# JianCao92/speaker-diarization

Measured on AMD Instinct MI355X. Metric: diarized audio throughput (CD gw/BIC + CL hi/BIC), higher is better.
Workload: dtype f64

## Files before the change

speaker-diarization_amd/csrc/spkd_cd.hpp:

```cpp
#pragma once
#include <type_traits>
#include "spkd_device.hpp"
#include "spkd_quad.hpp"
#include "spkd_stats.hpp"
#include "spkd_cluster.hpp"
#include "../../include/spkd.h"

namespace spkd {

constexpr double NEG_MAXINT_M1 = -9223372036854775808.0;

struct TurnDesc {
    int64_t begin;
    int64_t len;
    int64_t cand_off;
    int64_t cand_cap;
    int64_t ev_off;
    int64_t ev_cap;
    int64_t id;
};

struct BestD {
    double d;
    long long k;
// ... 269 lines not shown
                load_fv<G::BR>(xi + f * DA, a);
                load_fv<G::BC>(xj + f * DA, b);
                frame(a, b);
            }
        }
        pos = stop;
    }
#ifdef SPKD_PROFILE
    SW_TICK(0);
    if (tid == 0) for (int i = 0; i < 3; ++i) atomicAdd(&g_gw_prof[8 + i], sw_acc[i]);
    if (tid == 0) atomicAdd(&g_gw_prof[11], sw_reached);
#endif
}

struct SweepOut {
    long long pos;
    double next_i;
    long long built_k;
};

template <int NW>
__device__ __noinline__ SweepOut gw_sweep_coarse(const float* __restrict__ fr, double* __restrict__ cache,
                                                 double start, double istep, double built_i,
                                                 long long built_k, long long cap, long long sweep_pos,
                                                 long long c, int fresh, int* err) {
    using G = Gw<NW>;
    extern __shared__ double gw_lds[];
    double* ldsEnd = gw_lds;
    float* xs = (float*)(gw_lds + TREC);
    const int tid = threadIdx.x;
    const SweepLane SL = sweep_lane<NW>(tid);
    const SPKD_GLOBAL float* gfr = (const SPKD_GLOBAL float*)fr;
    SPKD_GLOBAL double* gcache = (SPKD_GLOBAL double*)cache;
    double acc[G::NACC];
    if (fresh) {
#pragma unroll
        for (int e = 0; e < G::NACC; ++e) acc[e] = 0.0;
    } else {
        sweep_gather_lds<NW>(ldsEnd, SL, acc);
    }
    __syncthreads();
    auto next_stop = [&]() -> long long {
        const long long b = built_k < cap ? (long long)(start + built_i) : c;
        return b < c ? b : c;
    };
    gw_sweep<NW>(gfr, xs, SL, tid, acc, sweep_pos, next_stop(), c, [&](long long pos) -> long long {
        if (pos < c) {
            sweep_dump_packed<NW>(gcache + built_k * REC, SL, acc);
            ++built_k;
            built_i += istep;
            return next_stop();
        }
        sweep_dump_lds<NW>(ldsEnd, SL, acc);
        return -1;
    }, err);
    SweepOut o;
    o.pos = c;
    o.next_i = built_i;
    o.built_k = built_k;
    return o;
}

template <int NW>
__device__ __noinline__ void gw_sweep_fine(const float* __restrict__ fr, double* __restrict__ cache,
                                           const double* __restrict__ base, long long base_pos,
                                           double start, double fine_i0, long long F,
                                           long long first_slot, int* err) {
    using G = Gw<NW>;
    extern __shared__ double gw_lds[];
    float* xs = (float*)(gw_lds + TREC);
    const int tid = threadIdx.x;
    const SweepLane SL = sweep_lane<NW>(tid);
    const SPKD_GLOBAL float* gfr = (const SPKD_GLOBAL float*)fr;
    SPKD_GLOBAL double* gcache = (SPKD_GLOBAL double*)cache;
    double acc[G::NACC];
#pragma unroll
    for (int e = 0; e < G::NACC; ++e) acc[e] = 0.0;
    if (base) sweep_gather_packed<NW>((const SPKD_GLOBAL double*)base, SL, acc);
    double fx = fine_i0;
    long long fk = 0;
    const long long last = (long long)(start + (fine_i0 + (double)(F - 1)));
    gw_sweep<NW>(gfr, xs, SL, tid, acc, base_pos, (long long)(start + fx), last, [&](long long) -> long long {
        sweep_dump_packed<NW>(gcache + (first_slot + fk) * REC, SL, acc);
        ++fk;
        fx += 1;
        return fk < F ? (long long)(start + fx) : -1;
    }, err);
}

template <int NW>
__device__ __noinline__ void gw_sweep_tail(const float* __restrict__ fr, long long from, long long to,
                                           double* __restrict__ out, int* err) {
    using G = Gw<NW>;
    extern __shared__ double gw_lds[];
    float* xs = (float*)(gw_lds + TREC);
    const int tid = threadIdx.x;
    const SweepLane SL = sweep_lane<NW>(tid);
    const SPKD_GLOBAL float* gfr = (const SPKD_GLOBAL float*)fr;
    SPKD_GLOBAL double* gout = (SPKD_GLOBAL double*)out;
    double acc[G::NACC];
#pragma unroll
    for (int e = 0; e < G::NACC; ++e) acc[e] = 0.0;
    gw_sweep<NW>(gfr, xs, SL, tid, acc, from, to, to, [&](long long) -> long long {
        sweep_dump_packed<NW>(gout, SL, acc);
        return -1;
    }, err);
}

__device__ __forceinline__ void single_split_matrix(int pass, const double* ldsEnd,
                                                    const double* __restrict__ rec_b,
                                                    double n1, double n2, double (&q)[DA]) {
    const double n = n1 + n2;
    double rc[DA];
    if (pass == PASS_POOLED) {
        single_rows_from_tri(ldsEnd, q);
        cov_rows(q, n);
        return;
    }
    single_rows_from_packed(rec_b, q);
    if (pass == PASS_LEFT) {
        cov_rows(q, n1);
        return;
    }
    single_rows_from_tri(ldsEnd, rc);
    if (pass == PASS_RIGHT) {
#pragma unroll
        for (int j = 0; j < DA; ++j) q[j] = rc[j] - q[j];
        cov_rows(q, n2);
    } else {
        const double al1 = (n1 / n) / (n1 - 1.0), al2 = (n2 / n) / (n2 - 1.0);
        const double be1 = al1 / n1, be2 = al2 / n2;
        const double s1i = q[D], s2i = rc[D] - q[D];
#pragma unroll
        for (int j = 0; j < D; ++j) {
            const double q1 = q[j], q2 = rc[j] - q[j];
            const double s1j = readlane_d(s1i, j), s2j = readlane_d(s2i, j);
            double v = fma(al2, q2, al1 * q1);
            v = fma(-(be1 * s1i), s1j, v);
            q[j] = fma(-(be2 * s2i), s2j, v);
        }
    }
}

__device__ __forceinline__ double quad_split_det(int pass, bool two, const double* ldsEnd,
                                                    const double* __restrict__ rec_b,
                                                    double ik, double start, long long a, long long c,
                                                    const QuadLane& L, int* err) {
    QuadRows q;
    double svb[QS];
    PASS_T0();
    int ta = L.t;
    asm volatile("" : "+v"(ta));
    {
        const int t12 = ta < QL ? ta : QL - 1;
        const double* rt[2];
        long long o1 = 512;
        asm volatile("" : "+v"(o1));
        rt[0] = rec_b + t12;
        rt[1] = rt[0] + o1;
#pragma unroll
        for (int s = 0; s < QS; ++s) {
#pragma unroll
            for (int j = 0; j < tri_cols(s); ++j) {
                const int e = pk_off(j) + QL * s - j;
                q.r[s][j] = rt[e / 512][e % 512];
            }
            const int c = QL * s + t12;
            svb[s] = rec_b[pk_off(c) + D - c];
        }
    }
    __builtin_amdgcn_sched_barrier(0);
    const long long b = pass == PASS_POOLED ? a : (long long)(start + ik);
    const double n1 = (double)(b - a), n2 = (double)(c - b);
    const double n = n1 + n2;
    double al, ga, k1a, k1c, k2a, k2c, w1, w2;
    {
        const bool glr = two && pass == PASS_GLR;
        double al1 = 0.0, al2 = 0.0, b1 = 0.0, b2 = 0.0;
        if (two) {
            al1 = (n1 / n) / (n1 - 1.0);
            al2 = (n2 / n) / (n2 - 1.0);
            b1 = al1 / n1;
            b2 = al2 / n2;
        }
        const double np = pass == PASS_RIGHT ? n2 : (pass == PASS_LEFT ? n1 : n);
        const double f = fast_recip(np - 1.0);
        const double sa = pass == PASS_RIGHT ? -1.0 : (pass == PASS_LEFT ? 1.0 : 0.0);
        const double sg = pass == PASS_LEFT ? 0.0 : 1.0;
        al = glr ? al1 - al2 : sa * f;
        ga = glr ? al2 : sg * f;
        k1a = glr ? 1.0 : sa;
        k1c = glr ? 0.0 : sg;
        w1 = glr ? -b1 : -(f * fast_recip(np));
        k2a = glr ? -1.0 : 0.0;
        k2c = glr ? 1.0 : 0.0;
        w2 = glr ? -b2 : 0.0;
    }
    __builtin_amdgcn_sched_barrier(0);
    PASS_LOADED();
    double v1[QS], v2[QS], c1[QS], c2[QS];
#pragma unroll
    for (int s = 0; s < QS; ++s) {
#pragma unroll
        for (int j = 0; j < tri_cols(s); ++j)
            q.r[s][j] = fma(ga, ldsEnd[(tri_off(s) + j) * 16 + ta], al * q.r[s][j]);
        const double sc = ldsEnd[(TREC_SUMS + s) * 16 + ta];
        v1[s] = fma(k1c, sc, k1a * svb[s]);
        v2[s] = fma(k2c, sc, k2a * svb[s]);
        c1[s] = w1 * v1[s];
        c2[s] = w2 * v2[s];
        __builtin_amdgcn_sched_barrier(0);
    }
    TriRank1<0>::run(q, c1, v1);
    if (two) TriRank1<0>::run(q, c2, v2);
    auto form_single = [&](int mi, double (&arr)[DA]) {
        const double* rm = (const double*)__shfl((unsigned long long)rec_b, 16 * mi);
        single_split_matrix(__shfl(pass, 16 * mi), ldsEnd, rm, __shfl(n1, 16 * mi), __shfl(n2, 16 * mi), arr);
    };
    const double det = tri_det(q, L.m, err, form_single);
    PASS_DONE();
    return det;
}


#ifdef SPKD_PROFILE
#define GW_TICK(i) do { const unsigned long long now_ = clock64(); prof_acc[i] += now_ - prof_t; prof_t = now_; } while (0)
#else
#define GW_TICK(i) ((void)0)
#endif

struct GwState {
    double start, end, ws, dws, cur_i, built_i, maxd, maxi, fine_i0;
    long long n_memo;
    long long n_written;
    long long C;
    long long built_k, sweep_pos;
    int fresh;
    long long best_k, F, base, count;
    long long seg_src, seg_dst;
    int nw, nd;
    int next_q;
    int fine;
    int go;
    int abort;
    int tail_in_lds;
};

template <int NW>
__global__ __launch_bounds__(Gw<NW>::TPB, NW == 8 ? 1 : 2) void k_gw(
        const float* __restrict__ frames, const TurnDesc* __restrict__ turns, spkd_cd_params P,
        double* __restrict__ cache_all, double* __restrict__ cand_all,
        int32_t* __restrict__ n_win, double* __restrict__ win_maxd, int32_t* __restrict__ win_det,
        double* __restrict__ det_start, double* __restrict__ det_maxi, double* __restrict__ det_d,
        double* __restrict__ final_start, double* __restrict__ seg_stats, spkd_cand_log* clog,
        long long log_cap, unsigned long long* log_count, int* err,
        double* pinv_ws) {
    extern __shared__ double gw_lds[];
    double* ldsEnd = gw_lds;
    constexpr int GW_WAVES = NW, GW_TPB = Gw<NW>::TPB;
    __shared__ BestD red[GW_WAVES];
    __shared__ double s_ldS;
    __shared__ double s_common[2];
    __shared__ GwState S;
    const int tid = threadIdx.x, lane = lane_id(), wave = tid >> 6;
    const QuadLane L = quad_lane();
    const TurnDesc T = turns[blockIdx.x];
    const int turn = (int)T.id;
    const long long n = T.len;
    const float* fr = frames + T.begin * D;
    double* cache = cache_all + T.cand_off * REC;
    const long long cap = T.cand_cap;
    double* c_i = cand_all + 4 * T.cand_off;
    double* c_left = c_i + cap;
    double* c_x = c_left + cap;
    double* c_w = c_x + cap;

#ifdef SPKD_PROFILE
    unsigned long long prof_acc[4] = {0ull, 0ull, 0ull, 0ull}, prof_t = clock64(), prof_scans = 0ull;
    unsigned long long prof_passes = 0ull, prof_items = 0ull;
#endif
    for (int e = tid; e < TREC; e += GW_TPB) ldsEnd[e] = 0.0;
    for (int e = tid; e < REC; e += GW_TPB) cache[e] = 0.0;

    const int kind = P.kind;
    const double winsize = P.winsize, winstep = P.winstep, rate = P.rate;
    const double minfeas = rate / 2;
    const double istep = rate / 10;
    const double fn = (double)n;
    const double pen_w = P.lambdac * 0.5 * PEN_UNIT;
    if (tid == 0) {
        S.start = 0.0;
        S.end = winsize * 2;
        S.ws = minfeas;
        S.dws = P.deltaws;
        S.cur_i = minfeas;
        S.built_i = minfeas;
        S.maxd = 0.0; S.maxi = 0.0; S.fine_i0 = 0.0;
        S.n_memo = 0; S.n_written = 0; S.C = 0;
        S.built_k = 0; S.sweep_pos = 0; S.fresh = 1;
        S.best_k = 0; S.F = 0; S.base = 0; S.count = 0;
        S.seg_src = -1; S.seg_dst = -1;
        S.nw = 0; S.nd = 0; S.fine = 0;
        S.go = (S.end <= fn) ? 1 : 0;
        S.abort = 0;
        S.tail_in_lds = 0;
    }
    __syncthreads();
    GW_TICK(0);

    while (S.go) {
        if (tid == 0) {
            if (!S.fine) {
                if (S.nw >= T.ev_cap) {
                    atomicOr(err, 4);
                    S.abort = 1;
                } else {
                    const double lim = S.end - S.start - minfeas;
                    double cur_i = S.cur_i;
                    long long C = S.C, n_written = S.n_written;
                    while (cur_i < lim) {
// ... 430 lines not shown
```

speaker-diarization_amd/csrc/spkd_cluster.hpp:

```cpp
#pragma once
#include "spkd_device.hpp"
#include "spkd_quad.hpp"
#include "spkd_tri.hpp"
#include "../../include/spkd.h"

namespace spkd {

constexpr double MAXINT_F = 9223372036854775808.0;
constexpr double PEN_UNIT = 39.0 + 0.5 * 39.0 * 40.0;
constexpr int AUX = 3 * DA;
constexpr int ERR_DEGENERATE_MERGE = 2;

__device__ __forceinline__ unsigned long long dkey(double v) {
    unsigned long long b = (unsigned long long)__double_as_longlong(v);
    return (b >> 63) ? ~b : (b | 0x8000000000000000ull);
}
__device__ __forceinline__ double dkey_inv(unsigned long long k) {
    unsigned long long b = (k >> 63) ? (k & 0x7fffffffffffffffull) : ~k;
    return __longlong_as_double((long long)b);
}
template <bool MAXOP>
__device__ __forceinline__ unsigned wave_red_u32(unsigned x) {
    auto op = [](unsigned a, unsigned b) { return MAXOP ? (a > b ? a : b) : (a < b ? a : b); };
    x = op(x, (unsigned)__builtin_amdgcn_update_dpp((int)x, (int)x, 0xB1, 0xf, 0xf, false));
    x = op(x, (unsigned)__builtin_amdgcn_update_dpp((int)x, (int)x, 0x4E, 0xf, 0xf, false));
    x = op(x, (unsigned)__builtin_amdgcn_update_dpp((int)x, (int)x, 0x141, 0xf, 0xf, false));
    x = op(x, (unsigned)__builtin_amdgcn_update_dpp((int)x, (int)x, 0x140, 0xf, 0xf, false));
    const unsigned a = (unsigned)__builtin_amdgcn_readlane((int)x, 0), b = (unsigned)__builtin_amdgcn_readlane((int)x, 16);
    const unsigned c = (unsigned)__builtin_amdgcn_readlane((int)x, 32), d = (unsigned)__builtin_amdgcn_readlane((int)x, 48);
    return op(op(a, b), op(c, d));
}
__device__ __forceinline__ int wave_scan_i32(int x) {
    x += __builtin_amdgcn_update_dpp(0, x, 0x111, 0xf, 0xf, false);
    x += __builtin_amdgcn_update_dpp(0, x, 0x112, 0xf, 0xf, false);
    x += __builtin_amdgcn_update_dpp(0, x, 0x114, 0xf, 0xf, false);
    x += __builtin_amdgcn_update_dpp(0, x, 0x118, 0xf, 0xf, false);
    x += __builtin_amdgcn_update_dpp(0, x, 0x142, 0xa, 0xf, false);
    x += __builtin_amdgcn_update_dpp(0, x, 0x143, 0xc, 0xf, false);
    return x;
}
template <bool MAXOP>
__device__ __forceinline__ unsigned long long wave_red_u64(unsigned long long k) {
    const unsigned hi = (unsigned)(k >> 32), lo = (unsigned)k;
    const unsigned h = wave_red_u32<MAXOP>(hi);
    const unsigned l = wave_red_u32<MAXOP>(hi == h ? lo : (MAXOP ? 0u : 0xffffffffu));
    return ((unsigned long long)h << 32) | l;
}
__device__ __forceinline__ void wave_argmin_key(unsigned long long key, unsigned idx,
                                                unsigned long long& okey, unsigned& oidx) {
    okey = wave_red_u64<false>(key);
    oidx = wave_red_u32<false>(key == okey ? idx : 0xffffffffu);
}

__device__ __forceinline__ bool stat_valid(double d) {
    return d == d && fabs(d) < __builtin_huge_val();
}

__device__ __forceinline__ double kl2_combine(double s1, double p1, double m1,
                                              double s2, double p2, double m2);
__device__ __forceinline__ double kl2_from_aux(const double* __restrict__ a1,
                                               const double* __restrict__ a2) {
    int i = lane_id();
    i = i >= D ? D - 1 : i;
    return kl2_combine(a1[i], a1[DA + i], a1[2 * DA + i], a2[i], a2[DA + i], a2[2 * DA + i]);
}
__device__ __forceinline__ double kl2_from_aux_serial(const double* a1, const double* a2) {
    double t1 = 0.0, t2 = 0.0;
    for (int i = 0; i < D; ++i) {
        const float dm = (float)a1[2 * DA + i] - (float)a2[2 * DA + i];
        const double delta = (double)dm;
        t1 += (a1[i] - a2[i]) * (a2[DA + i] - a1[DA + i]);
        t2 += ((a1[DA + i] + a2[DA + i]) * delta) * delta;
    }
    return 0.5 * t1 + 0.5 * t2;
}

__device__ __forceinline__ void kl2_lane_terms(double (&a)[DA], double mean_i,
                                               double& ds, double& dp, double& mu, double* pinv_ws) {
    double out[2];
    spd_diag_terms_fn(a, out, pinv_ws);
    ds = out[0];
    dp = out[1];
    mu = (double)(float)mean_i;
}

__device__ __forceinline__ double kl2_combine(double s1, double p1, double m1,
                                              double s2, double p2, double m2) {
    const float dm = (float)m1 - (float)m2;
    const double delta = (double)dm;
    const double t1 = wave_sum39((s1 - s2) * (p2 - p1));
    const double t2 = wave_sum39(((p1 + p2) * delta) * delta);
    return 0.5 * t1 + 0.5 * t2;
}

constexpr int PT_WAVES = 4;

__device__ __forceinline__ void quadrec_from_packed(const double* __restrict__ g, double* __restrict__ o, int tid) {
    for (int e = tid; e < QREC; e += 256) {
        const int t = e & 15, sj = e >> 4;
        const int s = sj / DA, j = sj - s * DA;
        double v = 0.0;
        if (t < QL) {
            const int i = QL * s + t;
            const int r = i < j ? i : j, cc = i < j ? j : i;
            v = g[pk(r, cc)];
        } else if (e == QREC_COUNT_AT) {
            v = g[REC - 1];
        }
        o[e] = v;
    }
}

__global__ __launch_bounds__(256) void k_to_quadrec(const double* __restrict__ packed, int64_t n_rec,
                                                    double* __restrict__ qr) {
    const int64_t c = blockIdx.x;
    if (c >= n_rec) return;
    quadrec_from_packed(packed + c * REC, qr + c * QREC, threadIdx.x);
}

__device__ __forceinline__ void single_rows_from_packed(const double* __restrict__ rec, double (&q)[DA]) {
    int i = lane_id();
    i = i >= D ? D - 1 : i;
#pragma unroll
    for (int j = 0; j < D; ++j) q[j] = rec[j <= i ? pk_low(i, j) : pk_low(j, i)];
    q[D] = rec[pk_low(D, i)];
}

__device__ __forceinline__ void single_rows_from_qr(const double* __restrict__ qr, double (&q)[DA]) {
    int i = lane_id();
    i = i >= D ? D - 1 : i;
    const int base = (i / QL) * DA * 16 + (i % QL);
#pragma unroll
    for (int j = 0; j < DA; ++j) q[j] = qr[base + j * 16];
}

__device__ __forceinline__ void kl2_aux_from_qr(const double* qr, double* aux_out, double* pinv_ws) {
    double a[DA];
    single_rows_from_qr(qr, a);
    const double n = qr_count(qr);
    const double mean_i = a[D] / n;
    cov_rows(a, n);
    double ds, dp, mu;
    kl2_lane_terms(a, mean_i, ds, dp, mu, pinv_ws);
    const int lane = lane_id();
    if (lane < D) {
        aux_out[lane] = ds;
        aux_out[DA + lane] = dp;
        aux_out[2 * DA + lane] = mu;
    }
}

__device__ __forceinline__ void single_pair_matrix(int kind, const double* __restrict__ qrA,
                                                   const double* __restrict__ qrC, bool self,
                                                   double (&q)[DA]) {
    const double nA = qr_count(qrA);
    single_rows_from_qr(qrA, q);
    if (self) { cov_rows(q, nA); return; }
    const double nC = qr_count(qrC), n = nA + nC;
    double q2[DA];
    single_rows_from_qr(qrC, q2);
    if (kind == SPKD_BIC) {
#pragma unroll
        for (int j = 0; j < DA; ++j) q[j] += q2[j];
        cov_rows(q, n);
    } else {
        const double al1 = (nA / n) / (nA - 1.0), al2 = (nC / n) / (nC - 1.0);
        const double be1 = al1 / nA, be2 = al2 / nC;
        const double s1i = q[D], s2i = q2[D];
#pragma unroll
        for (int j = 0; j < D; ++j) {
            const double s1j = readlane_d(s1i, j), s2j = readlane_d(s2i, j);
            double v = fma(al2, q2[j], al1 * q[j]);
            v = fma(-(be1 * s1i), s1j, v);
            q[j] = fma(-(be2 * s2i), s2j, v);
        }
    }
}

#ifdef SPKD_PROFILE
__device__ unsigned long long g_pass_prof[4];
#define PASS_T0() const unsigned long long pass_t0_ = clock64()
#define PASS_LOADED() asm volatile("s_waitcnt vmcnt(0)" ::: "memory"); const unsigned long long pass_t1_ = clock64()
#define PASS_DONE() do { if (lane_id() == 0 && ((pass_t0_ >> 4) & 63) == 0) { const unsigned long long pass_t2_ = clock64();  \
        atomicAdd(&g_pass_prof[0], pass_t1_ - pass_t0_); atomicAdd(&g_pass_prof[1], pass_t2_ - pass_t0_); \
        atomicAdd(&g_pass_prof[2], 1ull); } } while (0)
#else
#define PASS_T0() ((void)0)
#define PASS_LOADED() ((void)0)
#define PASS_DONE() ((void)0)
#endif

template <bool TWO>
__device__ __forceinline__ double quad_pair_det(int kind, const double* ldsA, double nA,
                                                   const double* __restrict__ gA,
                                                   const double* __restrict__ qrC,
                                                   const double* __restrict__ pkC, bool self,
                                                   const QuadLane& L, int* err, double nC_known = -1.0) {
    const double nC = self ? 0.0 : (nC_known >= 0.0 ? nC_known : pkC[REC - 1]);
    const double n = nA + nC;
    const bool glr = TWO && (kind == SPKD_GLR && !self);
    const double f = fast_recip(n - 1.0);
    double wa = f, wc = self ? 0.0 : f;
    double k1 = -(f * fast_recip(n)), k2 = 0.0;
    if constexpr (TWO) {
        if (glr) {
            wa = (nA / n) / (nA - 1.0);
            wc = (nC / n) / (nC - 1.0);
            k1 = -(wa / nA);
            k2 = -(wc / nC);
        }
    }
    int ta = L.t;
    asm volatile("" : "+v"(ta));
    QuadRows q;
    double sc[QS];
    PASS_T0();
    {
        const int t12 = ta < QL ? ta : QL - 1;
        const double* rt[2];
        long long o1 = 512;
        asm volatile("" : "+v"(o1));
        rt[0] = pkC + t12;
        rt[1] = rt[0] + o1;
#pragma unroll
        for (int s = 0; s < QS; ++s) {
#pragma unroll
            for (int j = 0; j < tri_cols(s); ++j) {
                const int e = pk_off(j) + QL * s - j;
                q.r[s][j] = rt[e / 512][e % 512];
            }
            const int c = QL * s + t12;
            sc[s] = pkC[pk_off(c) + D - c];
        }
    }
    __builtin_amdgcn_sched_barrier(0);
    PASS_LOADED();
    double v1[QS], v2[QS], c1[QS], c2[QS];
#pragma unroll
    for (int s = 0; s < QS; ++s) {
#pragma unroll
        for (int j = 0; j < tri_cols(s); ++j)
            q.r[s][j] = fma(wa, ldsA[(s * DA + j) * 16 + ta], wc * q.r[s][j]);
        const double sa = ldsA[(s * DA + D) * 16 + ta];
        const double scs = self ? 0.0 : sc[s];
        v1[s] = glr ? sa : sa + scs;
        v2[s] = glr ? scs : 0.0;
        c1[s] = k1 * v1[s];
        c2[s] = k2 * v2[s];
        __builtin_amdgcn_sched_barrier(0);
    }
    TriRank1<0>::run(q, c1, v1);
    if constexpr (TWO) TriRank1<0>::run(q, c2, v2);
    auto form_single = [&](int mi, double (&a)[DA]) {
        const double* rm = (const double*)__shfl((unsigned long long)qrC, 16 * mi);
        single_pair_matrix(kind, gA, rm, __shfl((int)self, 16 * mi) != 0, a);
    };
    const double det = tri_det(q, L.m, err, form_single);
    PASS_DONE();
    return det;
}

__device__ __forceinline__ void stage_record(double* lds, const double* __restrict__ g, int tid, int nthreads) {
    for (int e = tid; e < QREC; e += nthreads) lds[e] = g[e];
}

constexpr int PT2_WAVES = 2;

__device__ __forceinline__ void quad_load_packed(const double* __restrict__ pkC, int ta, QuadRows& q, double (&sc)[QS]) {
    const int t12 = ta < QL ? ta : QL - 1;
    const double* rt[2];
    long long o1 = 512;
    asm volatile("" : "+v"(o1));
    rt[0] = pkC + t12;
    rt[1] = rt[0] + o1;
#pragma unroll
    for (int s = 0; s < QS; ++s) {
#pragma unroll
        for (int j = 0; j < tri_cols(s); ++j) {
            const int e = pk_off(j) + QL * s - j;
            q.r[s][j] = rt[e / 512][e % 512];
        }
        const int c = QL * s + t12;
        sc[s] = pkC[pk_off(c) + D - c];
    }
}

__device__ __forceinline__ void quad_from_packed_lds(double* lds, const double* __restrict__ g, int lane) {
    for (int e = lane; e < QREC; e += WAVE) {
        const int t = e & 15, sj = e >> 4;
        const int s = sj / DA, j = sj - s * DA;
        double v = 0.0;
        if (t < QL) {
            const int i = QL * s + t;
            const int r = i < j ? i : j, cc = i < j ? j : i;
            v = g[pk(r, cc)];
        } else if (e == QREC_COUNT_AT) {
            v = g[REC - 1];
        }
        lds[e] = v;
    }
}

__global__ __launch_bounds__(PT2_WAVES * WAVE) void k_pair_terms(
        const double* __restrict__ stats, const int32_t* __restrict__ ia,
        const int32_t* __restrict__ ib, int64_t n_pairs, int flags,
        double* __restrict__ out, int* err,
        double* pinv_ws) {
    __shared__ double slabs[PT2_WAVES][2][QREC];
    const int wave = threadIdx.x >> 6;
    const int lane = lane_id();
    const int64_t pair = (int64_t)blockIdx.x * PT2_WAVES + wave;
    if (pair >= n_pairs) return;
    double* ldsA = slabs[wave][0];
    double* ldsB = slabs[wave][1];
    const double* A = stats + (int64_t)ia[pair] * REC;
    const double* B = stats + (int64_t)ib[pair] * REC;
    const double n1 = A[REC - 1], n2 = B[REC - 1];
    const double n = n1 + n2;
    const QuadLane L = quad_lane();
    int ta = L.t;
    asm volatile("" : "+v"(ta));
    QuadRows q;
    double sc[QS];
    quad_load_packed(B, ta, q, sc);
    quad_from_packed_lds(ldsA, A, lane);
    quad_from_packed_lds(ldsB, B, lane);
    const bool want_glr = (flags & SPKD_WANT_GLR) != 0;
    const int mode = (L.m == 3 && !want_glr) ? 2 : L.m;
    double wa, wc, k1a, k1c, w1, k2c, w2;
    {
        const double fA = 1.0 / (n1 - 1.0), fB = 1.0 / (n2 - 1.0), fU = 1.0 / (n - 1.0);
        const double al1 = (n1 / n) / (n1 - 1.0), al2 = (n2 / n) / (n2 - 1.0);
        wa = mode == 0 ? fA : (mode == 1 ? 0.0 : (mode == 2 ? fU : al1));
        wc = mode == 0 ? 0.0 : (mode == 1 ? fB : (mode == 2 ? fU : al2));
        k1a = mode == 1 ? 0.0 : 1.0;
        k1c = (mode == 1 || mode == 2) ? 1.0 : 0.0;
        w1 = mode == 0 ? -(fA / n1) : (mode == 1 ? -(fB / n2) : (mode == 2 ? -(fU / n) : -(al1 / n1)));
        k2c = mode == 3 ? 1.0 : 0.0;
        w2 = mode == 3 ? -(al2 / n2) : 0.0;
    }
    double v1[QS], v2[QS], c1[QS], c2[QS];
#pragma unroll
    for (int s = 0; s < QS; ++s) {
#pragma unroll
        for (int j = 0; j < tri_cols(s); ++j)
            q.r[s][j] = fma(wa, ldsA[(s * DA + j) * 16 + ta], wc * q.r[s][j]);
        const double sa = ldsA[(s * DA + D) * 16 + ta];
        v1[s] = fma(k1c, sc[s], k1a * sa);
        v2[s] = k2c * sc[s];
        c1[s] = w1 * v1[s];
        c2[s] = w2 * v2[s];
        __builtin_amdgcn_sched_barrier(0);
    }
    TriRank1<0>::run(q, c1, v1);
    TriRank1<0>::run(q, c2, v2);
    auto form_single = [&](int mi, double (&a)[DA]) {
        const int md = (mi == 3 && !want_glr) ? 2 : mi;
        if (md == 0) single_pair_matrix(SPKD_BIC, ldsA, ldsA, true, a);
        else if (md == 1) single_pair_matrix(SPKD_BIC, ldsB, ldsB, true, a);
        else single_pair_matrix(md == 2 ? SPKD_BIC : SPKD_GLR, ldsA, ldsB, false, a);
    };
    const double ld = log(tri_det(q, L.m, err, form_single));
    double res[4];
#pragma unroll
    for (int mi = 0; mi < 4; ++mi) res[mi] = __shfl(ld, 16 * mi);
    double kl = __builtin_nan("");
    if (flags & SPKD_WANT_KL2) {
        double* slab = ldsA;
        double a[DA];
        double ds[2], dp[2], mu[2];
#pragma unroll 1
        for (int t = 0; t < 2; ++t) {
            stage1(slab, t ? B : A);
            row_from_slab(slab, a);
            const double nn = t ? n2 : n1;
            const double mean_i = a[D] / nn;
            cov_rows(a, nn);
            kl2_lane_terms(a, mean_i, ds[t], dp[t], mu[t], pinv_ws);
        }
        kl = kl2_combine(ds[0], dp[0], mu[0], ds[1], dp[1], mu[1]);
    }
    if (lane == 0) {
        double* o = out + pair * 8;
        o[0] = n1; o[1] = n2; o[2] = res[0]; o[3] = res[1]; o[4] = res[2];
        o[5] = want_glr ? res[3] : __builtin_nan("");
        o[6] = kl; o[7] = 0.0;
    }
}

__device__ __forceinline__ void cluster_prep_block(
        const double* __restrict__ qr, int64_t n_rec, int kind,
        double* __restrict__ ld, double* __restrict__ aux, int* err,
        double* pinv_ws, int64_t block) {
    const int wave = threadIdx.x >> 6;
    const int64_t w = block * PT_WAVES + wave;
    if (kind == SPKD_KL2) {
        if (w >= n_rec) return;
        kl2_aux_from_qr(qr + w * QREC, aux + w * AUX, pinv_ws);
        if (lane_id() == 0) ld[w] = 0.0;
        return;
    }
    if (w * 4 >= n_rec) return;
    const QuadLane L = quad_lane();
    const double* recs[4];
    bool selfs[4];
#pragma unroll
    for (int mi = 0; mi < 4; ++mi) {
        int64_t c = w * 4 + mi;
        c = c < n_rec ? c : n_rec - 1;
        recs[mi] = qr + c * QREC;
        selfs[mi] = true;
    }
    int64_t c = w * 4 + L.m;
    const bool valid = c < n_rec;
    c = valid ? c : n_rec - 1;
    const double* R = qr + c * QREC;
    QuadRows q;
    double sv[QS];
    const double nR = qr_count(R), fR = fast_recip(nR - 1.0);
    quad_load_scaled(R, L.t, fR, q, sv);
    double c1[QS];
    const double gR = -(fR * fast_recip(nR));
#pragma unroll
    for (int s = 0; s < QS; ++s) c1[s] = gR * sv[s];
    TriRank1<0>::run(q, c1, sv);
    auto form_single = [&](int mi, double (&a)[DA]) { single_pair_matrix(kind, recs[mi], recs[mi], true, a); };
    const double v = tri_logdet(q, L.m, err, form_single);
    if (valid && L.t == 0) ld[c] = v;
}

__global__ __launch_bounds__(PT_WAVES * WAVE) void k_cluster_prep(
        const double* __restrict__ qr, int64_t n_rec, int kind,
        double* __restrict__ ld, double* __restrict__ aux, int* err,
        double* pinv_ws) {
    cluster_prep_block(qr, n_rec, kind, ld, aux, err, pinv_ws, blockIdx.x);
}

__global__ __launch_bounds__(PT_WAVES * WAVE) void k_cluster_prep_batch(
        const double* __restrict__ qr, const int64_t* __restrict__ seg_off, int kind,
        double* __restrict__ ld, double* __restrict__ aux, int* prob_err,
        double* pinv_ws) {
    const int64_t off = seg_off[blockIdx.x];
    cluster_prep_block(qr + off * QREC, seg_off[blockIdx.x + 1] - off, kind, ld + off, aux + off * AUX,
                       prob_err + blockIdx.x, pinv_ws, blockIdx.y);
}

// ... 1056 lines not shown
```

speaker-diarization_amd/csrc/spkd_quad.hpp:

```cpp
#pragma once
#include "spkd_device.hpp"

namespace spkd {

constexpr int QL = 13;
constexpr int QS = 3;

struct QuadRows {
    double r[QS][D];
};

template <int K>
__device__ __forceinline__ double bcast16(double v) {
    const long long x = __double_as_longlong(v);
    return __longlong_as_double(__builtin_amdgcn_update_dpp(0ll, x, 0x150 + K, 0xf, 0xf, true));
}

__device__ __forceinline__ double fast_recip(double x) {
    double r = __builtin_amdgcn_rcp(x);
    r = fma(fma(-x, r, 1.0), r, r);
    r = fma(fma(-x, r, 1.0), r, r);
    return r;
}

}

namespace spkd {

constexpr int QREC = QS * DA * 16;
constexpr int QREC_COUNT_AT = (0 * DA + D) * 16 + 15;

__host__ __device__ constexpr int qr_index(int i, int j) { return ((i / QL) * DA + j) * 16 + (i % QL); }

struct QuadLane {
    int m;
    int t;
};

__device__ __forceinline__ QuadLane quad_lane() {
    QuadLane L;
    const int lane = lane_id();
    L.m = lane >> 4;
    L.t = lane & 15;
    return L;
}

__device__ __forceinline__ double qr_count(const double* __restrict__ qr) { return qr[QREC_COUNT_AT]; }

__device__ __forceinline__ void quad_load_scaled(const double* __restrict__ qr, int t, double w,
                                                 QuadRows& q, double (&sv)[QS]) {
#pragma unroll
    for (int s = 0; s < QS; ++s) {
#pragma unroll
        for (int j = 0; j < D; ++j) q.r[s][j] = w * qr[(s * DA + j) * 16 + t];
        sv[s] = qr[(s * DA + D) * 16 + t];
    }
}


constexpr int TLINES = 3 * QL + 3 * QL + 3;
constexpr int TREC = TLINES * 16;
constexpr int TREC_SUMS = 6 * QL;
constexpr int TREC_COUNT_AT = TREC_SUMS * 16 + 15;
__host__ __device__ constexpr int tri_off(int s) { return s == 0 ? 0 : (s == 1 ? QL : 3 * QL); }

__device__ __forceinline__ int tri_slot(int r, int j) {
    if (r < D) { const int s = r / QL; return (tri_off(s) + j) * 16 + (r - QL * s); }
    if (j < D) { const int s = j / QL; return (TREC_SUMS + s) * 16 + (j - QL * s); }
    return TREC_COUNT_AT;
}


__device__ __forceinline__ int tri_image_source(int idx) {
    const int t = idx & 15, line = idx >> 4;
    if (line >= TREC_SUMS) {
        const int s = line - TREC_SUMS;
        if (t < QL) return pk_low(D, QL * s + t);
        return idx == TREC_COUNT_AT ? REC - 1 : -1;
    }
    if (t >= QL) return -1;
    const int s = line < QL ? 0 : (line < 3 * QL ? 1 : 2);
    const int j = line - tri_off(s);
    const int r = QL * s + t;
    return r >= j ? pk_low(r, j) : pk_low(j, r);
}


}
```

speaker-diarization_amd/csrc/spkd_tri.hpp:

```cpp
#pragma once
#include "spkd_quad.hpp"

namespace spkd {

__host__ __device__ constexpr int tri_cols(int s) { return QL * (s + 1); }

template <int T, bool NOP>
__device__ __forceinline__ void fmac_bcast16(double& acc, double src, double m) {
    if constexpr (NOP)
        asm volatile("s_nop 1\n\tv_fmac_f64_dpp %0, %1, %2 row_newbcast:%3 row_mask:0xf bank_mask:0xf"
                     : "+v"(acc) : "v"(src), "v"(m), "n"(T));
    else
        asm volatile("v_fmac_f64_dpp %0, %1, %2 row_newbcast:%3 row_mask:0xf bank_mask:0xf"
                     : "+v"(acc) : "v"(src), "v"(m), "n"(T));
}

template <int T, bool NOP = true>
__device__ __forceinline__ double bcast16_nop(double v) {
    double r;
    if constexpr (NOP)
        asm volatile("s_nop 1\n\tv_mov_b64_dpp %0, %1 row_newbcast:%2 row_mask:0xf bank_mask:0xf"
                     : "=v"(r) : "v"(v), "n"(T));
    else
        asm volatile("v_mov_b64_dpp %0, %1 row_newbcast:%2 row_mask:0xf bank_mask:0xf"
                     : "=v"(r) : "v"(v), "n"(T));
    return r;
}

#ifndef SPKD_TRI_COLNOP
#define SPKD_TRI_COLNOP 0
#endif
template <int K, int J>
struct TriCol {
    static __device__ __forceinline__ void run(QuadRows& q, const double (&l)[QS]) {
        if constexpr (J < D) {
            constexpr int SJ = J / QL, TJ = J % QL;
            fmac_bcast16<TJ, SPKD_TRI_COLNOP != 0>(q.r[SJ][J], q.r[SJ][K], l[SJ]);
#pragma unroll
            for (int s = SJ + 1; s < QS; ++s) fmac_bcast16<TJ, false>(q.r[s][J], q.r[SJ][K], l[s]);
            TriCol<K, J + 1>::run(q, l);
        }
    }
};

struct PivotChain {
    double piv, r, e;
};

constexpr int NEWTON_OPS = 3;
constexpr int CHAIN_OPS = 3 + NEWTON_OPS + QS;

struct DetAcc {
    double det;
    int sign;
};

template <int P, int OP>
__device__ __forceinline__ void chain_op(QuadRows& q, PivotChain& ch, double (&ln)[QS], DetAcc& da, double piv_cur) {
    constexpr int S = P / QL, T = P % QL;
    if constexpr (OP == 0) {
        constexpr int have = (QS - 1 - S) + 1;
        if constexpr (P == 0 || have < 2)
            asm volatile("s_nop %3\n\tv_mov_b64_dpp %0, %1 row_newbcast:%2 row_mask:0xf bank_mask:0xf"
                         : "=v"(ch.piv) : "v"(q.r[S][P]), "n"(T), "n"(P == 0 ? 1 : 1 - have));
        else
            asm volatile("v_mov_b64_dpp %0, %1 row_newbcast:%2 row_mask:0xf bank_mask:0xf"
                         : "=v"(ch.piv) : "v"(q.r[S][P]), "n"(T));
    } else if constexpr (OP == 1) {
        if constexpr (P > 0) {
            da.det *= piv_cur;
            da.sign |= __double2hiint(piv_cur);
        }
    } else if constexpr (OP == 2) {
        ch.r = __builtin_amdgcn_rcp(ch.piv);
    } else if constexpr (OP < 3 + NEWTON_OPS) {
        if constexpr (OP == 3) ch.e = fma(-ch.piv, ch.r, 1.0);
        else if constexpr (OP == 4) ch.e = fma(ch.e, ch.e, ch.e);
        else ch.r = fma(ch.r, ch.e, ch.r);
    } else {
        constexpr int s = OP - 3 - NEWTON_OPS;
        if constexpr (s >= S) ln[s] = -q.r[s][P] * ch.r;
        else ln[s] = 0.0;
    }
    __builtin_amdgcn_sched_barrier(0);
}

template <int P, int OP>
__device__ __forceinline__ void chain_rest(QuadRows& q, PivotChain& ch, double (&ln)[QS], DetAcc& da, double piv_cur) {
    if constexpr (OP < CHAIN_OPS) {
        chain_op<P, OP>(q, ch, ln, da, piv_cur);
        chain_rest<P, OP + 1>(q, ch, ln, da, piv_cur);
    }
}

template <int K, int J, int OP>
struct TriColAhead {
    static __device__ __forceinline__ void run(QuadRows& q, const double (&l)[QS], PivotChain& ch, double (&ln)[QS],
                                               DetAcc& da, double piv_k) {
        if constexpr (J < D) {
            constexpr int SJ = J / QL, TJ = J % QL;
            fmac_bcast16<TJ, false>(q.r[SJ][J], q.r[SJ][K], l[SJ]);
#pragma unroll
            for (int s = SJ + 1; s < QS; ++s) fmac_bcast16<TJ, false>(q.r[s][J], q.r[SJ][K], l[s]);
            constexpr int first = K + 1;
            constexpr int avail = D - 1 - first;
            constexpr int gap = avail >= 2 * CHAIN_OPS ? 2 : 1;
            constexpr bool emit = OP < CHAIN_OPS && ((J - first) % gap == 0);
            if constexpr (emit) {
                __builtin_amdgcn_sched_barrier(0);
                chain_op<K + 1, OP>(q, ch, ln, da, piv_k);
            }
            TriColAhead<K, J + 1, emit ? OP + 1 : OP>::run(q, l, ch, ln, da, piv_k);
        } else {
            __builtin_amdgcn_sched_barrier(0);
            chain_rest<K + 1, OP>(q, ch, ln, da, piv_k);
        }
    }
};

struct NoHook {
    template <int K> __device__ __forceinline__ void after_step() {}
    __device__ __forceinline__ void redo() {}
};

template <int K>
struct TriStepAhead {
    template <class Hook>
    static __device__ __forceinline__ void run(QuadRows& q, DetAcc& da, const double (&l)[QS], double piv_k, Hook& hook) {
        if constexpr (K + 1 < D) {
            PivotChain ch;
            double ln[QS];
            TriColAhead<K, K + 1, 0>::run(q, l, ch, ln, da, piv_k);
            hook.template after_step<K>();
            TriStepAhead<K + 1>::run(q, da, ln, ch.piv, hook);
        } else {
            da.det *= piv_k;
            da.sign |= __double2hiint(piv_k);
            hook.template after_step<K>();
        }
    }
};

template <class Hook>
__device__ __forceinline__ bool tri_det_nopivot(QuadRows& q, double& det_out, Hook& hook) {
    DetAcc da;
    da.det = 1.0;
    da.sign = 0;
    PivotChain ch;
    double l0[QS];
    __builtin_amdgcn_sched_barrier(0);
    chain_rest<0, 0>(q, ch, l0, da, 1.0);
    TriStepAhead<0>::run(q, da, l0, ch.piv, hook);
    det_out = da.det;
    return (da.sign >= 0) && (da.det == da.det) && (da.det < __builtin_huge_val());
}

__device__ __forceinline__ bool tri_det_nopivot(QuadRows& q, double& det_out) {
    NoHook h;
    return tri_det_nopivot(q, det_out, h);
}

template <int J>
struct TriRank1 {
    static __device__ __forceinline__ void run(QuadRows& q, const double (&c)[QS], const double (&v)[QS]) {
        if constexpr (J < D) {
            constexpr int SJ = J / QL, TJ = J % QL;
            fmac_bcast16<TJ, true>(q.r[SJ][J], v[SJ], c[SJ]);
#pragma unroll
            for (int s = SJ + 1; s < QS; ++s) fmac_bcast16<TJ, false>(q.r[s][J], v[SJ], c[s]);
            TriRank1<J + 1>::run(q, c, v);
        }
    }
};

template <class FormSingle, class Hook>
__device__ __forceinline__ double tri_det(QuadRows& q, int m, int* err, FormSingle form_single, Hook& hook) {
    double det;
    const bool ok = tri_det_nopivot(q, det, hook);
    const unsigned long long badmask = __ballot(!ok);
    if (badmask) {
#pragma unroll 1
        for (int mi = 0; mi < 4; ++mi) {
            if (((badmask >> (16 * mi)) & 0xffffull) == 0ull) continue;
            double a[DA];
            form_single(mi, a);
            const double v = det_pivoted_fn(a, err);
            if (m == mi) det = v;
        }
        hook.redo();
    }
    return det;
}

template <class FormSingle>
__device__ __forceinline__ double tri_det(QuadRows& q, int m, int* err, FormSingle form_single) {
    NoHook h;
    return tri_det(q, m, err, form_single, h);
}

template <class FormSingle>
__device__ __forceinline__ double tri_logdet(QuadRows& q, int m, int* err, FormSingle form_single) {
    return log(tri_det(q, m, err, form_single));
}

}
```

Before: 1443.

## Split quad row slots unevenly to shrink per-lane triangular storage

Replaces the fixed 13/13/13 split of the 39 matrix rows across three lane slots with a configurable uneven split at bases 0, 7 and 23, giving slots of 7, 16 and 16 rows. Because slot s keeps only tri_cols(s) columns, each lane now holds 7+23+39 columns instead of 13+26+39. The aim is fewer live registers and fewer broadcast FMAs in the triangular determinant. All index helpers, record layouts and load paths are generalised to match, with static_asserts guarding record bounds. The cost is that all 16 lanes of each group are now used by two slots, which may change load patterns and slot balance.

```diff
diff --git a/speaker-diarization_amd/csrc/spkd_cd.hpp b/speaker-diarization_amd/csrc/spkd_cd.hpp
--- a/speaker-diarization_amd/csrc/spkd_cd.hpp
+++ b/speaker-diarization_amd/csrc/spkd_cd.hpp
@@ -445,7 +445,7 @@
     int ta = L.t;
     asm volatile("" : "+v"(ta));
     {
-        const int t12 = ta < QL ? ta : QL - 1;
+        const int t12 = quad_load_lane(ta);
         const double* rt[2];
         long long o1 = 512;
         asm volatile("" : "+v"(o1));
@@ -455,10 +455,10 @@
         for (int s = 0; s < QS; ++s) {
 #pragma unroll
             for (int j = 0; j < tri_cols(s); ++j) {
-                const int e = pk_off(j) + QL * s - j;
+                const int e = quad_pk_at(s, j);
                 q.r[s][j] = rt[e / 512][e % 512];
             }
-            const int c = QL * s + t12;
+            const int c = quad_row(s, t12);
             svb[s] = rec_b[pk_off(c) + D - c];
         }
     }
diff --git a/speaker-diarization_amd/csrc/spkd_cluster.hpp b/speaker-diarization_amd/csrc/spkd_cluster.hpp
--- a/speaker-diarization_amd/csrc/spkd_cluster.hpp
+++ b/speaker-diarization_amd/csrc/spkd_cluster.hpp
@@ -100,8 +100,8 @@
         const int t = e & 15, sj = e >> 4;
         const int s = sj / DA, j = sj - s * DA;
         double v = 0.0;
-        if (t < QL) {
-            const int i = QL * s + t;
+        if (t < quad_rows(s)) {
+            const int i = quad_row(s, t);
             const int r = i < j ? i : j, cc = i < j ? j : i;
             v = g[pk(r, cc)];
         } else if (e == QREC_COUNT_AT) {
@@ -129,7 +129,7 @@
 __device__ __forceinline__ void single_rows_from_qr(const double* __restrict__ qr, double (&q)[DA]) {
     int i = lane_id();
     i = i >= D ? D - 1 : i;
-    const int base = (i / QL) * DA * 16 + (i % QL);
+    const int base = qr_index(i, 0);
 #pragma unroll
     for (int j = 0; j < DA; ++j) q[j] = qr[base + j * 16];
 }
@@ -216,7 +216,7 @@
     double sc[QS];
     PASS_T0();
     {
-        const int t12 = ta < QL ? ta : QL - 1;
+        const int t12 = quad_load_lane(ta);
         const double* rt[2];
         long long o1 = 512;
         asm volatile("" : "+v"(o1));
@@ -226,10 +226,10 @@
         for (int s = 0; s < QS; ++s) {
 #pragma unroll
             for (int j = 0; j < tri_cols(s); ++j) {
-                const int e = pk_off(j) + QL * s - j;
+                const int e = quad_pk_at(s, j);
                 q.r[s][j] = rt[e / 512][e % 512];
             }
-            const int c = QL * s + t12;
+            const int c = quad_row(s, t12);
             sc[s] = pkC[pk_off(c) + D - c];
         }
     }
@@ -267,7 +267,7 @@
 constexpr int PT2_WAVES = 2;
 
 __device__ __forceinline__ void quad_load_packed(const double* __restrict__ pkC, int ta, QuadRows& q, double (&sc)[QS]) {
-    const int t12 = ta < QL ? ta : QL - 1;
+    const int t12 = quad_load_lane(ta);
     const double* rt[2];
     long long o1 = 512;
     asm volatile("" : "+v"(o1));
@@ -277,10 +277,10 @@
     for (int s = 0; s < QS; ++s) {
 #pragma unroll
         for (int j = 0; j < tri_cols(s); ++j) {
-            const int e = pk_off(j) + QL * s - j;
+            const int e = quad_pk_at(s, j);
             q.r[s][j] = rt[e / 512][e % 512];
         }
-        const int c = QL * s + t12;
+        const int c = quad_row(s, t12);
         sc[s] = pkC[pk_off(c) + D - c];
     }
 }
@@ -290,8 +290,8 @@
         const int t = e & 15, sj = e >> 4;
         const int s = sj / DA, j = sj - s * DA;
         double v = 0.0;
-        if (t < QL) {
-            const int i = QL * s + t;
+        if (t < quad_rows(s)) {
+            const int i = quad_row(s, t);
             const int r = i < j ? i : j, cc = i < j ? j : i;
             v = g[pk(r, cc)];
         } else if (e == QREC_COUNT_AT) {
diff --git a/speaker-diarization_amd/csrc/spkd_quad.hpp b/speaker-diarization_amd/csrc/spkd_quad.hpp
--- a/speaker-diarization_amd/csrc/spkd_quad.hpp
+++ b/speaker-diarization_amd/csrc/spkd_quad.hpp
@@ -3,8 +3,40 @@
 
 namespace spkd {
 
-constexpr int QL = 13;
 constexpr int QS = 3;
+
+#ifndef SPKD_QUAD_BASES
+#define SPKD_QUAD_BASES 0, 7, 23
+#endif
+__host__ __device__ constexpr int quad_base_pick(int s, int b0, int b1, int b2) {
+    return s <= 0 ? b0 : (s == 1 ? b1 : (s == 2 ? b2 : D));
+}
+__host__ __device__ constexpr int quad_base(int s) { return quad_base_pick(s, SPKD_QUAD_BASES); }
+__host__ __device__ constexpr int quad_rows(int s) { return quad_base(s + 1) - quad_base(s); }
+__host__ __device__ constexpr int quad_row(int s, int t) { return quad_base(s) + t; }
+__host__ __device__ constexpr int quad_slot(int r) { return r >= quad_base(2) ? 2 : (r >= quad_base(1) ? 1 : 0); }
+__host__ __device__ constexpr int quad_lane_of(int r) { return r - quad_base(quad_slot(r)); }
+__host__ __device__ constexpr int tri_cols(int s) { return quad_base(s + 1); }
+
+constexpr int QLANES = quad_rows(0) > quad_rows(1) ? (quad_rows(0) > quad_rows(2) ? quad_rows(0) : quad_rows(2))
+                                                   : (quad_rows(1) > quad_rows(2) ? quad_rows(1) : quad_rows(2));
+static_assert(quad_base(0) == 0 && quad_rows(0) > 0 && quad_rows(1) > 0 && quad_rows(2) > 0 && QLANES <= 16, "slot bases");
+static_assert(quad_rows(0) < 16, "lane 15 of slot 0 holds the frame count");
+
+__host__ __device__ constexpr int quad_pk_at(int s, int j) { return pk_off(j) + quad_base(s) - j; }
+__device__ __forceinline__ int quad_load_lane(int t) {
+    if constexpr (QLANES < 16) return t < QLANES ? t : QLANES - 1;
+    else return t;
+}
+constexpr bool quad_loads_in_record() {
+    for (int s = 0; s < QS; ++s) {
+        if (quad_base(s) + QLANES - 1 >= D) return false;
+        for (int j = 0; j < tri_cols(s); ++j)
+            if (quad_pk_at(s, j) < 0 || quad_pk_at(s, j) + QLANES - 1 >= REC) return false;
+    }
+    return true;
+}
+static_assert(quad_loads_in_record(), "a packed load of some (slot, column, lane) leaves the record");
 
 struct QuadRows {
     double r[QS][D];
@@ -30,7 +62,7 @@
 constexpr int QREC = QS * DA * 16;
 constexpr int QREC_COUNT_AT = (0 * DA + D) * 16 + 15;
 
-__host__ __device__ constexpr int qr_index(int i, int j) { return ((i / QL) * DA + j) * 16 + (i % QL); }
+__host__ __device__ constexpr int qr_index(int i, int j) { return (quad_slot(i) * DA + j) * 16 + quad_lane_of(i); }
 
 struct QuadLane {
     int m;
@@ -58,30 +90,40 @@
 }
 
 
-constexpr int TLINES = 3 * QL + 3 * QL + 3;
+__host__ __device__ constexpr int tri_off(int s) {
+    return s <= 0 ? 0 : (s == 1 ? tri_cols(0) : (s == 2 ? tri_cols(0) + tri_cols(1) : tri_cols(0) + tri_cols(1) + tri_cols(2)));
+}
+constexpr int TREC_SUMS = tri_off(QS);
+constexpr int TLINES = TREC_SUMS + QS;
 constexpr int TREC = TLINES * 16;
-constexpr int TREC_SUMS = 6 * QL;
 constexpr int TREC_COUNT_AT = TREC_SUMS * 16 + 15;
-__host__ __device__ constexpr int tri_off(int s) { return s == 0 ? 0 : (s == 1 ? QL : 3 * QL); }
 
+__host__ __device__ constexpr int tri_row_at(int r) {
+    return r + (r >= quad_base(2) ? tri_off(2) * 16 - quad_base(2) : (r >= quad_base(1) ? tri_off(1) * 16 - quad_base(1) : 0));
+}
+__host__ __device__ constexpr int tri_sum_at(int j) {
+    return TREC_SUMS * 16 + j + (j >= quad_base(2) ? 32 - quad_base(2) : (j >= quad_base(1) ? 16 - quad_base(1) : 0));
+}
 __device__ __forceinline__ int tri_slot(int r, int j) {
-    if (r < D) { const int s = r / QL; return (tri_off(s) + j) * 16 + (r - QL * s); }
-    if (j < D) { const int s = j / QL; return (TREC_SUMS + s) * 16 + (j - QL * s); }
+    if (r < D) return tri_row_at(r) + 16 * j;
+    if (j < D) return tri_sum_at(j);
     return TREC_COUNT_AT;
 }
+static_assert(tri_row_at(quad_row(1, 2)) == (tri_off(1) * 16 + 2) && tri_row_at(quad_row(2, 15 < quad_rows(2) ? 15 : 0)) == tri_off(2) * 16 + (15 < quad_rows(2) ? 15 : 0)
+              && tri_sum_at(quad_row(2, 1)) == (TREC_SUMS + 2) * 16 + 1, "tri record index");
 
 
 __device__ __forceinline__ int tri_image_source(int idx) {
     const int t = idx & 15, line = idx >> 4;
     if (line >= TREC_SUMS) {
         const int s = line - TREC_SUMS;
-        if (t < QL) return pk_low(D, QL * s + t);
+        if (t < quad_rows(s)) return pk_low(D, quad_row(s, t));
         return idx == TREC_COUNT_AT ? REC - 1 : -1;
     }
-    if (t >= QL) return -1;
-    const int s = line < QL ? 0 : (line < 3 * QL ? 1 : 2);
+    const int s = line < tri_off(1) ? 0 : (line < tri_off(2) ? 1 : 2);
+    if (t >= quad_rows(s)) return -1;
     const int j = line - tri_off(s);
-    const int r = QL * s + t;
+    const int r = quad_row(s, t);
     return r >= j ? pk_low(r, j) : pk_low(j, r);
 }
 
diff --git a/speaker-diarization_amd/csrc/spkd_tri.hpp b/speaker-diarization_amd/csrc/spkd_tri.hpp
--- a/speaker-diarization_amd/csrc/spkd_tri.hpp
+++ b/speaker-diarization_amd/csrc/spkd_tri.hpp
@@ -2,8 +2,6 @@
 #include "spkd_quad.hpp"
 
 namespace spkd {
-
-__host__ __device__ constexpr int tri_cols(int s) { return QL * (s + 1); }
 
 template <int T, bool NOP>
 __device__ __forceinline__ void fmac_bcast16(double& acc, double src, double m) {
@@ -34,7 +32,7 @@
 struct TriCol {
     static __device__ __forceinline__ void run(QuadRows& q, const double (&l)[QS]) {
         if constexpr (J < D) {
-            constexpr int SJ = J / QL, TJ = J % QL;
+            constexpr int SJ = quad_slot(J), TJ = quad_lane_of(J);
             fmac_bcast16<TJ, SPKD_TRI_COLNOP != 0>(q.r[SJ][J], q.r[SJ][K], l[SJ]);
 #pragma unroll
             for (int s = SJ + 1; s < QS; ++s) fmac_bcast16<TJ, false>(q.r[s][J], q.r[SJ][K], l[s]);
@@ -57,7 +55,7 @@
 
 template <int P, int OP>
 __device__ __forceinline__ void chain_op(QuadRows& q, PivotChain& ch, double (&ln)[QS], DetAcc& da, double piv_cur) {
-    constexpr int S = P / QL, T = P % QL;
+    constexpr int S = quad_slot(P), T = quad_lane_of(P);
     if constexpr (OP == 0) {
         constexpr int have = (QS - 1 - S) + 1;
         if constexpr (P == 0 || have < 2)
@@ -98,7 +96,7 @@
     static __device__ __forceinline__ void run(QuadRows& q, const double (&l)[QS], PivotChain& ch, double (&ln)[QS],
                                                DetAcc& da, double piv_k) {
         if constexpr (J < D) {
-            constexpr int SJ = J / QL, TJ = J % QL;
+            constexpr int SJ = quad_slot(J), TJ = quad_lane_of(J);
             fmac_bcast16<TJ, false>(q.r[SJ][J], q.r[SJ][K], l[SJ]);
 #pragma unroll
             for (int s = SJ + 1; s < QS; ++s) fmac_bcast16<TJ, false>(q.r[s][J], q.r[SJ][K], l[s]);
@@ -164,7 +162,7 @@
 struct TriRank1 {
     static __device__ __forceinline__ void run(QuadRows& q, const double (&c)[QS], const double (&v)[QS]) {
         if constexpr (J < D) {
-            constexpr int SJ = J / QL, TJ = J % QL;
+            constexpr int SJ = quad_slot(J), TJ = quad_lane_of(J);
             fmac_bcast16<TJ, true>(q.r[SJ][J], v[SJ], c[SJ]);
 #pragma unroll
             for (int s = SJ + 1; s < QS; ++s) fmac_bcast16<TJ, false>(q.r[s][J], v[SJ], c[s]);
```

New measurement: 1526, median of 6. 1.06x the previous value.
